# catec/leica_point_cloud_processing

Hardware: AMD Instinct MI355X
Metric: GICP iterations/sec, 5M<->5M scan-vs-CAD (PCL-1.8.1-faithful BFGS GICP) (higher is better)
Workload: dtype f32 transform / f64 accumulate

## Files before the change

### include/mi355x_gicp_debug.h

```cpp
#ifndef MI355X_GICP_DEBUG_H
#define MI355X_GICP_DEBUG_H

#include "mi355x_gicp.h"

#ifdef __cplusplus
extern "C" {
#endif

int mgicp_debug_covariances(mgicp_ctx* ctx, int which, double* out_c6);
int mgicp_debug_source_order(mgicp_ctx* ctx, uint32_t* out, size_t cap);
int mgicp_debug_correspondences(mgicp_ctx* ctx, const float T_cm[16], int* out_tgt, double* out_M6);
int mgicp_debug_correspondences_seeded(mgicp_ctx* ctx, const float T_cm[16], int* out_tgt, double* out_M6);
int mgicp_debug_fdf(mgicp_ctx* ctx, const double x[6], double* f, double g6[6]);
int mgicp_debug_fdf_sums(mgicp_ctx* ctx, const double x[6], double out16[16]);
int mgicp_debug_fdf_sums_run(mgicp_ctx* ctx, const double* xs, int n, double* out16n);
int mgicp_debug_pass_bench(mgicp_ctx* ctx, const double x[6], int npasses, int mode, double* out_ms,
                           double out16[16]);
int mgicp_debug_moments(mgicp_ctx* ctx, const float T_cm[16], double out80[80]);
int mgicp_debug_supers(mgicp_ctx* ctx, int kind, const double* arg, double* out, int cap);
int mgicp_debug_finish_supers(mgicp_ctx* ctx, int nv, const double* rows, long long nsup, long long maxsup,
                              int nranks, double* out);
int mgicp_debug_wave_reduce(mgicp_ctx* ctx, const double* in, int nwaves, double* out_tree, double* out_rs);
int mgicp_debug_trace(mgicp_ctx* ctx, float* out, int max_iters);
#define MGICP_KERNEL_FAMILIES 6
int mgicp_debug_kernel_times(mgicp_ctx* ctx, double out_ms[MGICP_KERNEL_FAMILIES],
                             int out_counts[MGICP_KERNEL_FAMILIES]);
int mgicp_debug_pass_stats(mgicp_ctx* ctx, long long out[9]);
int mgicp_debug_server_time(mgicp_ctx* ctx, double* out_ms, long long* out_passes, long long* out_launches,
                            int reset);
int mgicp_debug_target_cov_slice(mgicp_ctx* ctx, int nranks, int rank, double* out_c6);
int mgicp_debug_vlist_stats(mgicp_ctx* ctx, long long out[8]);
int mgicp_debug_vlist_layout(mgicp_ctx* ctx, double out[24], uint8_t* state, uint32_t* length, uint32_t* offset,
                             size_t cap);
int mgicp_debug_match_stats(mgicp_ctx* ctx, long long out[8]);
int mgicp_set_profiling(mgicp_ctx* ctx, int on);
int mgicp_debug_option(mgicp_ctx* ctx, const char* name, double value);
int mgicp_debug_cache_stats(mgicp_ctx* ctx, long long out[5]);

#ifdef __cplusplus
}
#endif
#endif
// ... 1 lines not shown
```

### leica_point_cloud_processing_amd/_lib.py

```python
from __future__ import annotations

import ctypes
import os
import re

_HERE = os.path.dirname(os.path.abspath(__file__))
LIB_PATH = os.path.join(_HERE, os.environ.get("MGICP_LIB_NAME", "libmgicp.so"))
HEADER_PATH = os.path.join(os.path.dirname(_HERE), "include", "mi355x_gicp.h")
DEBUG_HEADER_PATH = os.path.join(os.path.dirname(_HERE), "include", "mi355x_gicp_debug.h")

MGICP_OK = 0
MGICP_E_INVALID = -1
MGICP_E_TOO_FEW_POINTS = -2
MGICP_E_SOLVER = -3
MGICP_E_NONFINITE = -4
MGICP_E_HIP = -5
MGICP_E_COMM = -6
MGICP_E_NOMEM = -7

MGICP_SOLVER_PCL_BFGS = 0
MGICP_SOLVER_GN = 1
MGICP_KERNEL_FAMILIES = 6


# ... 122 lines not shown
    "mgicp_fpfh_features": (ctypes.c_int, [_P, _P, _SZ, _SZ, _P, _SZ, _P, _SZ, ctypes.c_double, _P, _SZ, _P, _P,
                                            ctypes.POINTER(MgicpFpfhInfo)]),
    "mgicp_match_features": (ctypes.c_int, [_P, _P, _SZ, _SZ, _P, _SZ, _SZ, ctypes.c_double, _P, _P,
                                             ctypes.POINTER(_SZ), ctypes.POINTER(MgicpMatchInfo)]),
    "mgicp_segment_differences": (ctypes.c_int, [_P, _FP, _P, _SZ, _SZ, _P, _SZ, _SZ, ctypes.c_double, _P,
                                                  ctypes.POINTER(_SZ)]),
    "mgicp_voxel_grid": (ctypes.c_int, [_P, _P, _SZ, _SZ, ctypes.c_int, _DP, ctypes.c_int, _P, _SZ,
                                         ctypes.POINTER(_SZ)]),
    "mgicp_euclidean_clusters": (ctypes.c_int, [_P, _P, _SZ, _SZ, ctypes.c_double, _SZ, _SZ, _P, _P, _P,
                                                 ctypes.POINTER(MgicpClusterInfo)]),
    "mgicp_get_unique_id": (ctypes.c_int, [ctypes.c_char_p]),
    "mgicp_comm_init": (ctypes.c_int, [_P, ctypes.c_int, ctypes.c_int, ctypes.c_char_p]),
    "mgicp_comm_attach_shm": (ctypes.c_int, [_P, ctypes.c_char_p, _SZ]),
    "mgicp_comm_attach_xgmi": (ctypes.c_int, [_P, ctypes.c_int]),
    "mgicp_debug_pass_stats": (ctypes.c_int, [_P, ctypes.POINTER(ctypes.c_longlong)]),
    "mgicp_debug_server_time": (ctypes.c_int, [_P, _DP, ctypes.POINTER(ctypes.c_longlong),
                                               ctypes.POINTER(ctypes.c_longlong), ctypes.c_int]),
    "mgicp_debug_target_cov_slice": (ctypes.c_int, [_P, ctypes.c_int, ctypes.c_int, _DP]),
    "mgicp_debug_vlist_stats": (ctypes.c_int, [_P, ctypes.POINTER(ctypes.c_longlong)]),
    "mgicp_debug_match_stats": (ctypes.c_int, [_P, ctypes.POINTER(ctypes.c_longlong)]),
    "mgicp_debug_vlist_layout": (ctypes.c_int, [_P, _DP, _P, _P, _P, _SZ]),
    "mgicp_debug_source_order": (ctypes.c_int, [_P, ctypes.c_void_p, ctypes.c_size_t]),
    "mgicp_debug_covariances": (ctypes.c_int, [_P, ctypes.c_int, _DP]),
    "mgicp_debug_correspondences": (ctypes.c_int, [_P, _FP, _IP, _DP]),
    "mgicp_debug_correspondences_seeded": (ctypes.c_int, [_P, _FP, _IP, _DP]),
    "mgicp_debug_fdf": (ctypes.c_int, [_P, _DP, _DP, _DP]),
    "mgicp_debug_fdf_sums": (ctypes.c_int, [_P, _DP, _DP]),
    "mgicp_debug_fdf_sums_run": (ctypes.c_int, [_P, _DP, ctypes.c_int, _DP]),
    "mgicp_debug_pass_bench": (ctypes.c_int, [_P, _DP, ctypes.c_int, ctypes.c_int, _DP, _DP]),
    "mgicp_debug_moments": (ctypes.c_int, [_P, _FP, _DP]),
# ... 75 lines not shown
```

### leica_point_cloud_processing_amd/csrc/mgicp_ctx.hpp

```cpp
#pragma once
#include <hip/hip_runtime.h>
#include <rccl/rccl.h>

#include <algorithm>
#include <chrono>
#include <cstdio>
#include <cstdlib>
#include <cstring>
#include <memory>
#include <mutex>
#include <string>
#include <vector>

#include "../../include/mi355x_gicp.h"
#include "mgicp_internal.hpp"
#include "pass_memo.hpp"
#include "pcl_bfgs.hpp"
#include "shm_rows.hpp"

using namespace mgicp;

namespace mgicp {

constexpr int kFdfMaxBlocks = 512;
// ... 206 lines not shown
  bool srv_degraded = false;
  unsigned long long srv_next = 0;
  int cus = 0;
  int srv_cus = 0;
  int stall_pass = -1;
  int quit_pass = -1;
  double row_deadline_ms = 500.0;
  double remote_deadline_s = 120.0;
  unsigned long long* h_ptimes = nullptr;
  unsigned long long* d_ptimes = nullptr;
  bool host_rows = true;
  unsigned long long* h_rows = nullptr;
  unsigned long long* d_rows = nullptr;
  size_t rows_cap = 0;
  std::vector<double> row_sums;
  unsigned int pass_idx = 0;
  unsigned long long gather_idx = 0;
  bool have_shm = false;
  shm::Segment shm;
  bool have_xgmi = false;
  DevBuf<unsigned long long> xrows;
  std::vector<void*> xpeer;
  unsigned long long* h_xtot = nullptr;
  unsigned long long* d_xtot = nullptr;
  unsigned int* h_xgen = nullptr;
  unsigned int* d_xgen = nullptr;
  unsigned int xgen = 0;
  unsigned long long xseq = 0;
  hipStream_t xstream = nullptr;
  bool xstream_own = false;
// ... 22 lines not shown
  bool qperm_aux = false;
  DevBuf<uint32_t> aq_keys, aq_keys_sorted, aq_vals;
  DevBuf<unsigned char> aq_scratch;
  DevBuf<unsigned int> aux_cnt;
  DevBuf<uint32_t> knn_fb2;
  bool knn_wave = true;
  bool knn_logged = true;
  DevBuf<uint32_t> knn_fb;
  unsigned int knn_fallbacks = 0;
  DevBuf<float> fpartial;
  unsigned long long match_pairs_per_launch = kMatchPairsPerLaunch;
  long long match_stats[8] = {0, 0, 0, 0, 0, 0, 0, 0};
  bool vlist = true;
  bool fuse_compact = true;
  DevBuf<uint32_t> vl_defer;
  bool vl_stats = false;
  bool vl_valid = false;
  bool vl_alloc = false;
  bool vl_off = false;
  VListView vl{};
  size_t vl_ncells = 0;
  DevBuf<uint32_t> vl_cell, vl_build, vl_bcentre, vl_pend;
  DevBuf<float4> vl_pool;
  DevBuf<unsigned int> vl_ctr;
  uint32_t vl_epoch = 0;
  int vl_groups = 0;
  bool vl_eager = false;
  int vl_cold_groups = 2;
  size_t vl_pool_entries = 0;
  bool tcache_on = false;
// ... 86 lines not shown
  hipEvent_t e = nullptr;
  (void)hipEventCreate(&e);
  return e;
}

struct ProfScope {
  mgicp_ctx* ctx;
  int fam;
  hipEvent_t a = nullptr;
  ProfScope(mgicp_ctx* c, int f) : ctx(c), fam(f) {
    if (ctx->profiling && (fam != kFamFdf || (ctx->prof_tick++ % kProfStride) == 0)) {
      a = ev_get(ctx);
      (void)hipEventRecord(a, ctx->stream);
    }
  }
  ~ProfScope() {
    if (a) {
      hipEvent_t b = ev_get(ctx);
      (void)hipEventRecord(b, ctx->stream);
      ctx->pending.push_back({a, b, fam});
    }
  }
};

Mat4 apply_state(const Vec6& x);
void prof_resolve(mgicp_ctx* ctx);
void cancel_gated(mgicp_ctx* ctx);
void srv_resolve(mgicp_ctx* ctx);
void srv_release(mgicp_ctx* ctx);
int sync(mgicp_ctx* ctx);
int reset_stamps(mgicp_ctx* ctx);
int ensure_host_red(mgicp_ctx* ctx);
CorrSoA corr_soa(mgicp_ctx* ctx);
RowView row_view(const mgicp_ctx* ctx);
int ensure_rows(mgicp_ctx* ctx);
// ... 51 lines not shown
```

### leica_point_cloud_processing_amd/csrc/mgicp_debug.hip

```cpp
#pragma clang fp contract(off)

#include <algorithm>
#include <cstdio>
#include <cstring>
#include <mutex>
#include <string>
#include <vector>

#include "../../include/mi355x_gicp_debug.h"
#include "mgicp_ctx.hpp"

extern "C" {

int mgicp_debug_pass_stats(mgicp_ctx* ctx, long long out[9]) {
  if (!ctx || !out) return MGICP_E_INVALID;
  for (int i = 0; i < kStCount; ++i) out[i] = ctx->st[i];
  return MGICP_OK;
}

int mgicp_debug_server_time(mgicp_ctx* ctx, double* out_ms, long long* out_passes, long long* out_launches,
                            int reset) {
  if (!ctx || !out_ms || !out_passes || !out_launches) return MGICP_E_INVALID;
  *out_ms = ctx->srv_time_ms;
  *out_passes = ctx->srv_time_passes;
  *out_launches = ctx->srv_time_launches;
  if (reset) {
    ctx->srv_time_ms = 0;
    ctx->srv_time_passes = ctx->srv_time_launches = 0;
  }
  return MGICP_OK;
}
// ... 477 lines not shown
    ctx->src_lazy_ready = false;
  } else if (n == "knn_wave") {
    ctx->knn_wave = on;
  } else if (n == "knn_logged") {
    ctx->knn_logged = on;
    ctx->src.have_cov = ctx->tgt.have_cov = false;
    ctx->src_lazy_ready = false;
  } else if (n == "vlist") ctx->vlist = on, ctx->vl_valid = false;
  else if (n == "vlist_cold") ctx->vl_cold_groups = std::max(0, iv), ctx->vl_valid = false;
  else if (n == "vlist_eager") ctx->vl_eager = on, ctx->vl_valid = false;
  else if (n == "vlist_pool") {
    ctx->vl_pool_entries = value >= 1.0 ? static_cast<size_t>(std::min(value, 134217728.0)) : 0;
    ctx->vl_valid = false;
  } else if (n == "vlist_stats") ctx->vl_stats = on;
  else if (n == "fuse_compact") ctx->fuse_compact = on;
  else if (n == "target_cache") ctx->tcache_on = on;
  else if (n == "match_pairs_per_launch")
    ctx->match_pairs_per_launch = value >= 1.0 ? static_cast<unsigned long long>(std::min(value, 9.0e18)) : kMatchPairsPerLaunch;
  else if (n == "bar_cmd") {
    ctx->bar = on;
    if (!on && ctx->bar_cmd) {
      (void)hipFree(ctx->bar_cmd);
      ctx->bar_cmd = nullptr;
    }
    if (on && !ctx->bar_cmd) {
      hipDeviceProp_t prop;
      if (hipGetDeviceProperties(&prop, ctx->device) == hipSuccess && prop.isLargeBar &&
          hipExtMallocWithFlags(reinterpret_cast<void**>(&ctx->bar_cmd), sizeof(PassCmd), hipDeviceMallocFinegrained) ==
              hipSuccess)
        HIPCK(hipMemset(ctx->bar_cmd, 0, sizeof(PassCmd)));
// ... 11 lines not shown
```

### leica_point_cloud_processing_amd/csrc/mgicp_engine.hip

```cpp
#pragma clang fp contract(off)

#include <hip/hip_runtime.h>
#include <rccl/rccl.h>

#include <algorithm>
#include <cmath>
#include <cstdio>
#include <cstdlib>
#include <cstring>
#include <memory>
#include <string>
#include <thread>
#include <vector>

#include "host_upload.hpp"
#include "mgicp_ctx.hpp"
#include "gn_solver.hpp"

using namespace mgicp;

thread_local Graveyard* mgicp::t_new_ctx_grave = nullptr;

namespace {

// ... 95 lines not shown
  }
  ctx->vl.epoch = ctx->vl_epoch;
  ctx->vl.eager = ctx->vl_eager ? 1 : 0;
  ctx->vl.tpts = ctx->tgt.pts.p;
  return MGICP_OK;
}

bool sweep_listed(const mgicp_ctx* ctx) {
  return ctx->vlist && ctx->vl_valid && ctx->vl_alloc && !ctx->vl_off && ctx->vl_groups >= ctx->vl_cold_groups;
}

hipError_t launch_sweep(mgicp_ctx* ctx, const Mat4& T, double thr, bool seeded, const uint32_t* qp,
                        const FusedCompact* fc = nullptr) {
  const size_t p0 = ctx->shard_p0(), p1 = ctx->shard_p1();
  const GridView& g = ctx->tgt.view;
  if (sweep_listed(ctx))
    return launch_vl_sweep(g, ctx->vl, ctx->d_out, p0, p1, T.xf(), thr, seeded ? 1 : 0, ctx->prev_pos.p, ctx->flags.p,
                           ctx->cus, ctx->stream, fc);
  return launch_correspond_wave(g, ctx->d_out, p0, p1, T.xf(), thr, seeded ? 1 : 0, ctx->prev_pos.p, ctx->flags.p, qp,
                                ctx->stream);
}

int report_sweep(mgicp_ctx* ctx) {
  hipStream_t s = ctx->stream;
  if (ctx->vl_stats && sweep_listed(ctx)) {
    unsigned int c3[3];
    HIPCK(hipMemcpyAsync(c3, ctx->vl_ctr.p, 3 * sizeof(unsigned int), hipMemcpyDeviceToHost, s));
    HIPCK(ctx->u64.reserve(64));
    HIPCK(launch_vl_stats(ctx->vl, ctx->vl_ncells, ctx->u64.p, s));
    unsigned long long st[64];
// ... 36 lines not shown
                 ph[14], ph[15], ph[16], ph[17]);
  }
#endif
#if MGICP_CORR_STATS
  {
    unsigned long long st[8];
    HIPCK(hipStreamSynchronize(s));
    HIPCK(corr_stats_take(st));
    std::fprintf(stderr, "[corr-stats] wave scan: queries %llu accepted %llu rejected %llu | per-lane tests/query %.1f "
                 "ranges/query %.1f | lanes left to the per-lane search %llu | union-scan waves %llu of %llu, "
                 "candidates per union wave %.1f\n",
                 st[0], st[1], st[2], st[0] ? double(st[3]) / st[0] : 0.0, st[0] ? double(st[4]) / st[0] : 0.0, st[5],
                 st[7], (st[0] + 63) / 64, st[7] ? double(st[6]) / st[7] : 0.0);
  }
#endif
  return MGICP_OK;
}

struct AlignDrain {
  mgicp_ctx* ctx;
  bool armed = true;
  ~AlignDrain() {
    if (!armed) return;
    const std::string err = ctx->err;
    cancel_gated(ctx);
    (void)hipStreamSynchronize(ctx->stream);
    srv_release(ctx);
    if (!ctx->srv_ev.empty()) srv_resolve(ctx);
    ctx->err = err;
  }
// ... 210 lines not shown
  MGICP_TRACE_AT("corr: lists prepared");
  const bool fused = ctx->fuse_compact && sweep_listed(ctx) && ctx->tgt.have_cov &&
                     !ctx->tgt_cov_pending && !ctx->src_cov_pending &&
                     (ctx->src.have_cov || (ctx->lazy_src_cov && ctx->src_lazy_ready));
  FusedCompact fc{};
  if (fused) {
    HIPCK(ctx->vl_defer.reserve(std::max(chunk_count(ns), 1)));
    fc.cov_s = ctx->src.cov3();
    fc.cov_t = ctx->tgt.cov3();
    fc.R = rot_of(T, G);
    fc.cov_ok = ctx->src.have_cov ? nullptr : ctx->cov_ok.p;
    fc.ccnt = ctx->ccnt.p;
    fc.defer = ctx->vl_defer.p;
    fc.out = corr_soa(ctx);
  }
  {
    ProfScope ps(ctx, kFamCorr);
    HIPCK(launch_sweep(ctx, T, thr, seeded, qp, fused ? &fc : nullptr));
  }
  ctx->seed_valid = true;
  MGICP_TRACE_AT("corr: sweep queued");
  if (int rc = report_sweep(ctx)) return rc;
  {
    int rc = cov_join_all(ctx);
    if (rc) return rc;
    rc = cov_lazy(ctx);
    MGICP_TRACE_AT("corr: lazy covariances queued (sweep drained)");
    if (rc) return rc;
  }
  {
    ProfScope ps(ctx, kFamCompact);
    HIPCK(launch_compact(ctx->d_out, ctx->tgt.view.pts, ctx->src.cov3(), ctx->tgt.cov3(), rot_of(T, G),
                         ctx->prev_pos.p, ctx->flags.p, p0, p1, ctx->ccnt.p, corr_soa(ctx), s,
                         fused ? ctx->vl_defer.p : nullptr, fused ? ctx->vl_ctr.p + 3 : nullptr, ctx->cus));
  }
  ctx->have_corr = true;
  return MGICP_OK;
// ... 188 lines not shown
  ctx->tickets.release();
  ctx->tickets_n = 0;
  ctx->ccnt.release(); ctx->spart.release(); ctx->gath.release(); ctx->msuper.release();
  ctx->prev_pos.release(); ctx->flags.release();
  ctx->vl_cell.release(); ctx->vl_pool.release(); ctx->vl_ctr.release();
  ctx->vl_build.release(); ctx->vl_bcentre.release(); ctx->vl_pend.release(); ctx->vl_defer.release();
  ctx->cov_ok.release(); ctx->cov_need.release();
  ctx->aux_cnt.release(); ctx->knn_fb2.release();
  ctx->tpart.release();
  ctx->tpart_n = 0;
  ctx->corr_f.release(); ctx->corr_d.release();
  ctx->xyz_dev.release();
  if (ctx->mail) (void)hipFree(ctx->mail);
  if (ctx->h_red) (void)hipHostFree(ctx->h_red);
  if (ctx->h_cmd) (void)hipHostFree(ctx->h_cmd);
  if (ctx->h_gtrace) (void)hipHostFree(ctx->h_gtrace);
  if (ctx->h_ptimes) (void)hipHostFree(ctx->h_ptimes);
  if (ctx->h_rows) (void)hipHostFree(ctx->h_rows);
  xgmi_detach(ctx);
  if (ctx->xstream && ctx->xstream_own) (void)hipStreamDestroy(ctx->xstream);
  if (ctx->h_xtot) (void)hipHostFree(ctx->h_xtot);
  if (ctx->have_shm) {
    (void)hipHostUnregister(ctx->shm.base);
    shm::detach(ctx->shm);
    ctx->have_shm = false;
  }
  if (ctx->bar_cmd) (void)hipFree(ctx->bar_cmd);
  if (ctx->h_small) (void)hipHostFree(ctx->h_small);
  prof_resolve(ctx);
  srv_resolve(ctx);
// ... 135 lines not shown
```

### leica_point_cloud_processing_amd/csrc/mgicp_internal.hpp

```cpp
#pragma once
#include <hip/hip_runtime.h>
#include <cstddef>
#include <cstdint>

namespace mgicp {

struct GridView {
  float ox, oy, oz;
  float h, inv_h;
  float slop;
  int nx, ny, nz;
  const uint32_t* cell_start;
  const float4* pts;
  const uint8_t* empty_dist;
  const uint32_t* seed;
  const float4* pairs;
};

#ifndef MGICP_EMPTY_CAP
#define MGICP_EMPTY_CAP 15
#endif
constexpr int kEmptyCap = MGICP_EMPTY_CAP;

struct Cov3 {
// ... 91 lines not shown
  uint32_t* pend;
  uint32_t epoch;
  int eager;
};
struct FusedCompact {
  Cov3 cov_s, cov_t;
  Rot33d R;
  const uint8_t* cov_ok;
  uint32_t* ccnt;
  uint32_t* defer;
  CorrSoA out;
};
hipError_t launch_vl_sweep(const GridView& tgt, const VListView& vl, const float4* src, size_t p0, size_t p1,
                           Xf34 T, double thr, int seeded, uint32_t* nn_pos, uint32_t* flags, int cus,
                           hipStream_t s, const FusedCompact* fc = nullptr);
hipError_t launch_cov_need(const uint32_t* flags, uint8_t* cov_ok, size_t p0, size_t n, uint32_t* list,
                           unsigned int* count, hipStream_t s);
hipError_t launch_vl_stats(const VListView& vl, size_t ncells, unsigned long long* out , hipStream_t s);
size_t     pair_count(size_t n);
hipError_t launch_pairs(const float4* pts, size_t n, float4* out, hipStream_t s);
hipError_t launch_morton_keys(const float4* pts, size_t p0, size_t n, const float lo[3], float inv,
                              uint32_t* keys, uint32_t* vals, hipStream_t s);
hipError_t launch_compact(const float4* src, const float4* tpts, const Cov3& cov_s,
                          const Cov3& cov_t, Rot33d R, const uint32_t* nn_pos,
                          const uint32_t* flags, size_t p0, size_t p1, uint32_t* ccnt, CorrSoA out, hipStream_t s,
                          const uint32_t* defer = nullptr, const unsigned int* defer_count = nullptr, int cus = 0);
hipError_t launch_fdf_soa(const CorrSoA& c, const uint32_t* ccnt, size_t ns, Xf34 A,
                          double* partial, double* spart, int nb, unsigned int* tickets, double* out, int reverse,
                          unsigned long long* done_flag, unsigned long long seq, hipStream_t s,
                          unsigned long long* host_rows = nullptr, unsigned int rstamp = 0);
// ... 122 lines not shown
```

### leica_point_cloud_processing_amd/csrc/mgicp_kernels.hip

```cpp
#pragma clang fp contract(off)

#define MGICP_NN_UNROLL 4
#define MGICP_CORR_WAVES 8
#define MGICP_COV_WAVES 1
#ifndef MGICP_KNN_DIV
#define MGICP_KNN_DIV 0
#endif
#ifndef MGICP_CORR_STATS
#define MGICP_CORR_STATS 0
#endif
#define MGICP_SRV_STAGGER 2
#ifndef MGICP_VL_DIAG
#define MGICP_VL_DIAG 0
#endif
#ifndef MGICP_CORR_PHASES
#define MGICP_CORR_PHASES 0
#endif
constexpr int kRegListBatch = 8;

#include "mgicp_internal.hpp"

#include <hipcub/hipcub.hpp>

#include <algorithm>
// ... 1504 lines not shown
      o.sx[i] = s.x; o.sy[i] = s.y; o.sz[i] = s.z;
      o.qx[i] = w.x; o.qy[i] = w.y; o.qz[i] = w.z;
    }
  }
  if (deferred) {
    if (threadIdx.x == 0) defer[atomicAdd(&v.ctr[3], 1u)] = blockIdx.x;
    return;
  }
  if (threadIdx.x == 0) ccnt[blockIdx.x] = run;
  const uint32_t pad = ((run + 3u) & ~3u) - run;
  if (threadIdx.x < pad) {
    const size_t i = k0 + run + threadIdx.x;
    o.sx[i] = 0.f; o.sy[i] = 0.f; o.sz[i] = 0.f; o.qx[i] = 0.f; o.qy[i] = 0.f; o.qz[i] = 0.f;
    o.m00[i] = 0.0; o.m01[i] = 0.0; o.m02[i] = 0.0; o.m11[i] = 0.0; o.m12[i] = 0.0; o.m22[i] = 0.0;
  }
}

__global__ __launch_bounds__(256) void vl_centre_kernel(GridView tg, VListView v, double thr_c) {
  const unsigned int n = min(v.ctr[1], v.build_cap);
  for (unsigned int i = blockIdx.x * blockDim.x + threadIdx.x; i < n; i += gridDim.x * blockDim.x) {
    uint32_t ix, iy, iz;
    vl_cell_xyz(v, v.build[i], ix, iy, iz);
    const float cx = v.ox + (static_cast<float>(ix) + 0.5f) * v.c;
    const float cy = v.oy + (static_cast<float>(iy) + 0.5f) * v.c;
    const float cz = v.oz + (static_cast<float>(iz) + 0.5f) * v.c;
    NnVisitor vis;
    vis.init(cx, cy, cz, thr_c);
    seed_query(tg, 0, 0xffffffffu, cx, cy, cz, vis);
    if (vis.best != ~0ull) box_search(tg, cx, cy, cz, vis);
    else ring_search(tg, cx, cy, cz, vis);
// ... 2436 lines not shown
    case 25: return knn_cov_k<25>(g, eps, p0, p1, cov, perm, k, fb, fb_count, s, ring_cap, ok, chain, wave_handoff);
    case 30: return knn_cov_k<30>(g, eps, p0, p1, cov, perm, k, fb, fb_count, s, ring_cap, ok, chain, wave_handoff);
    default: break;
  }
  if (k < 1 || k > kMaxK) return hipErrorInvalidValue;
  if (k <= 8) return knn_cov_k<8>(g, eps, p0, p1, cov, perm, k, fb, fb_count, s, ring_cap, ok, chain, wave_handoff);
  if (k <= 16) return knn_cov_k<16>(g, eps, p0, p1, cov, perm, k, fb, fb_count, s, ring_cap, ok, chain, wave_handoff);
  if (k <= 24) return knn_cov_k<24>(g, eps, p0, p1, cov, perm, k, fb, fb_count, s, ring_cap, ok, chain, wave_handoff);
  return knn_cov_k<32>(g, eps, p0, p1, cov, perm, k, fb, fb_count, s, ring_cap, ok, chain, wave_handoff);
}


hipError_t launch_vl_sweep(const GridView& tgt, const VListView& vl, const float4* src, size_t p0, size_t p1,
                           Xf34 T, double thr, int seeded, uint32_t* nn_pos, uint32_t* flags, int cus,
                           hipStream_t s, const FusedCompact* fc) {
  if (p1 <= p0) return hipSuccess;
  hipError_t e = hipMemsetAsync(vl.ctr + 1, 0, 4 * sizeof(unsigned int), s);
  if (e != hipSuccess) return e;
  if (fc)
    vl_query_compact_kernel<<<chunk_count(p1 - p0), 256, 0, s>>>(vl, src, p0, p1 - p0, T, thr, nn_pos, flags, fc->cov_s,
                                                                  fc->cov_t, fc->R, fc->cov_ok, fc->ccnt, fc->defer,
                                                                  fc->out);
  else
    vl_query_kernel<<<nblk(p1 - p0), 256, 0, s>>>(vl, src, p0, p1 - p0, T, thr, nn_pos, flags);
  const double hd = std::sqrt(3.0) * (0.5 * static_cast<double>(vl.c) + static_cast<double>(vl.es));
  const double rc = vl.gate * (1.0 + 1e-5) + 1e-9 + hd;
  const unsigned g = static_cast<unsigned>(std::max(cus, 1));
  vl_centre_kernel<<<4 * g, 256, 0, s>>>(tgt, vl, rc * rc * (1.0 + 1e-5));
  vl_build_kernel<<<8 * g, 64 * kVlWavesS, 0, s>>>(tgt, vl);
  vl_build_large_kernel<<<4 * g, 64 * kVlWaves, 0, s>>>(tgt, vl);
  vl_fallback_kernel<<<8 * g, 256, 0, s>>>(tgt, vl, src, p0, T, thr, seeded, nn_pos, flags);
  return hipGetLastError();
}

constexpr int kCovNeedPer = 16;
__global__ __launch_bounds__(256) void cov_need_kernel(const uint32_t* __restrict__ flags, uint8_t* __restrict__ cov_ok,
                                                       size_t p0, size_t n, uint32_t* __restrict__ list,
                                                       unsigned int* __restrict__ count, int rest) {
  __shared__ unsigned int s_w[4];
// ... 700 lines not shown
      reinterpret_cast<const void*>(&knn_cov_kernel<32>),
      reinterpret_cast<const void*>(&knn_cov2_kernel<5>),
      reinterpret_cast<const void*>(&knn_cov2_kernel<10>),
      reinterpret_cast<const void*>(&knn_cov2_kernel<15>),
      reinterpret_cast<const void*>(&knn_cov2_kernel<20>),
      reinterpret_cast<const void*>(&knn_cov2_kernel<25>),
      reinterpret_cast<const void*>(&knn_cov2_kernel<30>),
      reinterpret_cast<const void*>(&knn_cov2_kernel<8>),
      reinterpret_cast<const void*>(&knn_cov2_kernel<16>),
      reinterpret_cast<const void*>(&knn_cov2_kernel<24>),
      reinterpret_cast<const void*>(&knn_cov2_kernel<32>),
      reinterpret_cast<const void*>(&morton_key_kernel),
      reinterpret_cast<const void*>(&chunk_compact_kernel),
      reinterpret_cast<const void*>(&chunk_compact_list_kernel),
      reinterpret_cast<const void*>(&vl_query_compact_kernel),
      reinterpret_cast<const void*>(&fdf_soa_kernel),
      reinterpret_cast<const void*>(&fdf_soa_gated_kernel),
      reinterpret_cast<const void*>(&fdf_server_kernel<false, kSrvWaves>),
      reinterpret_cast<const void*>(&fdf_server_kernel<true, kSrvWaves>),
      reinterpret_cast<const void*>(&fitness_kernel),
      reinterpret_cast<const void*>(&resolution_kernel),
      reinterpret_cast<const void*>(&radius_keep_kernel),
      reinterpret_cast<const void*>(&reduce_finish_kernel),
      reinterpret_cast<const void*>(&gn_moments_kernel),
      reinterpret_cast<const void*>(&publish_kernel),
      reinterpret_cast<const void*>(&super_reduce_kernel<kRedVals>),
      reinterpret_cast<const void*>(&super_reduce_kernel<kMomVals>),
      reinterpret_cast<const void*>(&finish_supers_kernel<kRedVals>),
      reinterpret_cast<const void*>(&finish_supers_kernel<kMomVals>),
      reinterpret_cast<const void*>(&finite_flags_kernel),
// ... 62 lines not shown
```

### leica_point_cloud_processing_amd/csrc/mgicp_pass.hip

```cpp
#pragma clang fp contract(off)

#include <hip/hip_runtime.h>
#include <rccl/rccl.h>

#include <algorithm>
#include <atomic>
#include <chrono>
#include <cmath>
#include <cstdio>
#include <cstring>

#include "mgicp_ctx.hpp"

using namespace mgicp;

namespace {

std::atomic<int> g_srv_busy[64];

struct Quat { float w, x, y, z; };
Quat quat_axis(float angle, int axis) {
  const float ha = 0.5f * angle;
  float s, c;
  ::sincosf(ha, &s, &c);
// ... 429 lines not shown
    {
      HIPCK(hipHostMalloc(reinterpret_cast<void**>(&ctx->h_ptimes), 2 * 1024 * sizeof(unsigned long long),
                          hipHostMallocMapped | hipHostMallocCoherent));
      HIPCK(hipHostGetDevicePointer(reinterpret_cast<void**>(&ctx->d_ptimes), ctx->h_ptimes, 0));
      std::memset(ctx->h_ptimes, 0, 2 * 1024 * sizeof(unsigned long long));
    }
    {
      HIPCK(hipHostMalloc(reinterpret_cast<void**>(&ctx->h_gtrace), 4 * 1024 * sizeof(unsigned long long),
                          hipHostMallocMapped | hipHostMallocCoherent));
      HIPCK(hipHostGetDevicePointer(reinterpret_cast<void**>(&ctx->d_gtrace), ctx->h_gtrace, 0));
      std::memset(ctx->h_gtrace, 0, 4 * 1024 * sizeof(unsigned long long));
      ctx->host_gt.assign(2 * 1024, 0.0);
    }
#endif
  }
  if (ctx->h_red) return MGICP_OK;
  HIPCK(hipHostMalloc(reinterpret_cast<void**>(&ctx->h_red), 2 * kRedVals * sizeof(double),
                      hipHostMallocMapped | hipHostMallocCoherent));
  HIPCK(hipHostGetDevicePointer(reinterpret_cast<void**>(&ctx->d_h_red), ctx->h_red, 0));
  std::memset(ctx->h_red, 0, 2 * kRedVals * sizeof(double));
  ctx->h_flag = reinterpret_cast<unsigned long long*>(ctx->h_red + kRedVals);
  ctx->d_flag = reinterpret_cast<unsigned long long*>(ctx->d_h_red + kRedVals);
  return MGICP_OK;
}

RowView mgicp::row_view(const mgicp_ctx* ctx) {
  RowView v;
  if (ctx->have_shm) {
    v.h0 = reinterpret_cast<unsigned long long*>(ctx->shm.rows(0));
    v.d0 = reinterpret_cast<unsigned long long*>(ctx->shm_d + ctx->shm.rows_offset_bytes());
// ... 60 lines not shown
        if (shm::row_complete(reinterpret_cast<const uint64_t*>(row), rstamp)) break;
        char msg[192];
        std::snprintf(msg, sizeof(msg),
                      "objective pass finished without publishing its super rows (row %lld of %lld: stamp %08x "
                      "expected, words 0 / 31 carry %08x / %08x)",
                      r, rv.nloc, rstamp, static_cast<unsigned int>(row[0] >> 32),
                      static_cast<unsigned int>(row[31] >> 32));
        return fail(ctx, MGICP_E_HIP, msg);
      }
      if (!own && el > ctx->remote_deadline_s)
        return fail(ctx, MGICP_E_COMM, "another rank did not publish its super rows (shared row segment)");
    }
    shm::row_decode(reinterpret_cast<const uint64_t*>(row), &ctx->row_sums[static_cast<size_t>(r) * kRedVals]);
    return MGICP_OK;
  };
  for (long long r = rv.first; r < rv.first + rv.nloc; ++r) {
    int rc = wait_row(r, true);
    if (rc) return rc;
  }
  t0 = std::chrono::steady_clock::now();
  for (long long r = 0; r < rv.ntot; ++r) {
    if (r >= rv.first && r < rv.first + rv.nloc) continue;
    int rc = wait_row(r, false);
    if (rc) return rc;
  }
  shm::fixed_total(ctx->row_sums.data(), rv.ntot, kRedVals, out);
  return MGICP_OK;
}

int mgicp::ensure_iter_buffers(mgicp_ctx* ctx) {
  const size_t ns = ctx->shard_p1() - ctx->shard_p0();
  const size_t nch = static_cast<size_t>(chunk_count(ns));
  const size_t msup = static_cast<size_t>(ctx->max_supers());
// ... 147 lines not shown
```

### leica_point_cloud_processing_amd/csrc/shm_rows.hpp

```cpp
#pragma once

#include <fcntl.h>
#include <sys/mman.h>
#include <sys/stat.h>
#include <unistd.h>

#include <atomic>
#include <cerrno>
#include <chrono>
#include <cstdint>
#include <cstring>
#include <string>
#include <thread>

namespace mgicp {
namespace shm {

constexpr uint64_t kMagic = 0x31574f5250434947ull;
constexpr int kMaxRanks = 64;
constexpr size_t kHeader = 4096;
constexpr size_t kFlagLine = 64;
constexpr size_t kRowWords = 32;
constexpr int kGathVals = 80;
constexpr size_t kIpcLine = 128;
// ... 161 lines not shown

inline void fixed_total(const double* rows, long long nsup, int nv, double* out) {
  for (int v = 0; v < nv; ++v) {
    double lanes[64];
    for (int l = 0; l < 64; ++l) {
      double a = 0.0;
      for (long long sg = l; sg < nsup; sg += 64) a += rows[static_cast<size_t>(sg) * nv + v];
      lanes[l] = a;
    }
    for (int off = 32; off > 0; off >>= 1)
      for (int i = 0; i < off; ++i) lanes[i] = lanes[i] + lanes[i + off];
    out[v] = lanes[0];
  }
}

inline bool gather_publish_wait(const Segment& s, uint64_t g, double timeout_s) {
  s.flag(s.rank)->store(g, std::memory_order_release);
  const auto t0 = std::chrono::steady_clock::now();
  for (int r = 0; r < s.nranks; ++r) {
    for (unsigned spins = 0; s.flag(r)->load(std::memory_order_acquire) < g; ++spins) {
      if ((spins & 1023u) == 1023u && elapsed_s(t0) > timeout_s) return false;
    }
  }
  return true;
}

}
}
```

### leica_point_cloud_processing_amd/engine.py

```python
from __future__ import annotations

import atexit
import ctypes

import numpy as np

from . import _lib
from .cloud import PointCloudRGB

DBL_MAX = float(np.finfo(np.float64).max)
_LIVE: set = set()
_SHUTTING_DOWN = [False]


@atexit.register
def _mark_shutdown():
    _SHUTTING_DOWN[0] = True


def _cm(T) -> np.ndarray:
    return np.ascontiguousarray(np.asarray(T, dtype=np.float32).T).reshape(16)


def _from_cm(buf) -> np.ndarray:
# ... 340 lines not shown
                    "comm_attach_shm")

    def attach_xgmi(self, on: bool = True):
        self._check(self._lib.mgicp_comm_attach_xgmi(self._h, int(bool(on))), "mgicp_comm_attach_xgmi")

    def detach_shm(self):
        self._check(self._lib.mgicp_comm_attach_shm(self._h, None, 0), "comm_attach_shm(detach)")

    PASS_STATS = ("server_launches", "server_passes", "launched_passes", "takeovers", "bar_commands",
                  "row_allocs", "transport", "server_denied", "memo_hits")

    def pass_stats(self) -> dict:
        out = (ctypes.c_longlong * len(self.PASS_STATS))()
        self._check(self._lib.mgicp_debug_pass_stats(self._h, out), "pass_stats")
        return {k: int(out[i]) for i, k in enumerate(self.PASS_STATS)}

    def server_time(self, reset: bool = False) -> dict:
        ms = ctypes.c_double()
        passes = ctypes.c_longlong()
        launches = ctypes.c_longlong()
        self._check(self._lib.mgicp_debug_server_time(self._h, ctypes.byref(ms), ctypes.byref(passes),
                                                      ctypes.byref(launches), int(reset)), "server_time")
        p = int(passes.value)
        return {"ms": ms.value, "passes": p, "launches": int(launches.value),
                "ms_per_pass": ms.value / p if p else None}

    def debug_target_cov_slice(self, nranks: int, rank: int, n_target: int) -> np.ndarray:
        out = np.zeros((max(1, -(-n_target // nranks)), 6), np.float64)
        cnt = self._check(self._lib.mgicp_debug_target_cov_slice(self._h, int(nranks), int(rank), _dp(out)),
                          "debug_target_cov_slice")
# ... 153 lines not shown
```

Before: 482.5.

## Skip follow-up sweep and covariance join when listed queries resolve all points

```diff
diff --git a/include/mi355x_gicp_debug.h b/include/mi355x_gicp_debug.h
--- a/include/mi355x_gicp_debug.h
+++ b/include/mi355x_gicp_debug.h
@@ -26,6 +26,7 @@
 int mgicp_debug_kernel_times(mgicp_ctx* ctx, double out_ms[MGICP_KERNEL_FAMILIES],
                              int out_counts[MGICP_KERNEL_FAMILIES]);
 int mgicp_debug_pass_stats(mgicp_ctx* ctx, long long out[9]);
+int mgicp_debug_round_stats(mgicp_ctx* ctx, long long out[4]);
 int mgicp_debug_server_time(mgicp_ctx* ctx, double* out_ms, long long* out_passes, long long* out_launches,
                             int reset);
 int mgicp_debug_target_cov_slice(mgicp_ctx* ctx, int nranks, int rank, double* out_c6);
diff --git a/leica_point_cloud_processing_amd/_lib.py b/leica_point_cloud_processing_amd/_lib.py
--- a/leica_point_cloud_processing_amd/_lib.py
+++ b/leica_point_cloud_processing_amd/_lib.py
@@ -160,6 +160,7 @@
     "mgicp_comm_attach_shm": (ctypes.c_int, [_P, ctypes.c_char_p, _SZ]),
     "mgicp_comm_attach_xgmi": (ctypes.c_int, [_P, ctypes.c_int]),
     "mgicp_debug_pass_stats": (ctypes.c_int, [_P, ctypes.POINTER(ctypes.c_longlong)]),
+    "mgicp_debug_round_stats": (ctypes.c_int, [_P, ctypes.POINTER(ctypes.c_longlong)]),
     "mgicp_debug_server_time": (ctypes.c_int, [_P, _DP, ctypes.POINTER(ctypes.c_longlong),
                                                ctypes.POINTER(ctypes.c_longlong), ctypes.c_int]),
     "mgicp_debug_target_cov_slice": (ctypes.c_int, [_P, ctypes.c_int, ctypes.c_int, _DP]),
diff --git a/leica_point_cloud_processing_amd/csrc/mgicp_ctx.hpp b/leica_point_cloud_processing_amd/csrc/mgicp_ctx.hpp
--- a/leica_point_cloud_processing_amd/csrc/mgicp_ctx.hpp
+++ b/leica_point_cloud_processing_amd/csrc/mgicp_ctx.hpp
@@ -244,6 +244,7 @@
   unsigned long long* d_rows = nullptr;
   size_t rows_cap = 0;
   std::vector<double> row_sums;
+  bool rows_running = true;
   unsigned int pass_idx = 0;
   unsigned long long gather_idx = 0;
   bool have_shm = false;
@@ -296,6 +297,12 @@
   bool vlist = true;
   bool fuse_compact = true;
   DevBuf<uint32_t> vl_defer;
+  bool round_fast = true;
+  unsigned long long* h_round = nullptr;
+  unsigned long long* d_round = nullptr;
+  unsigned int round_stamp = 0;
+  const unsigned int* vl_ctr_zero = nullptr;
+  long long round_st[4] = {0, 0, 0, 0};
   bool vl_stats = false;
   bool vl_valid = false;
   bool vl_alloc = false;
@@ -412,11 +419,13 @@
       (void)hipEventRecord(a, ctx->stream);
     }
   }
-  ~ProfScope() {
+  ~ProfScope() { close(); }
+  void close() {
     if (a) {
       hipEvent_t b = ev_get(ctx);
       (void)hipEventRecord(b, ctx->stream);
       ctx->pending.push_back({a, b, fam});
+      a = nullptr;
     }
   }
 };
diff --git a/leica_point_cloud_processing_amd/csrc/mgicp_debug.hip b/leica_point_cloud_processing_amd/csrc/mgicp_debug.hip
--- a/leica_point_cloud_processing_amd/csrc/mgicp_debug.hip
+++ b/leica_point_cloud_processing_amd/csrc/mgicp_debug.hip
@@ -15,6 +15,12 @@
 int mgicp_debug_pass_stats(mgicp_ctx* ctx, long long out[9]) {
   if (!ctx || !out) return MGICP_E_INVALID;
   for (int i = 0; i < kStCount; ++i) out[i] = ctx->st[i];
+  return MGICP_OK;
+}
+
+int mgicp_debug_round_stats(mgicp_ctx* ctx, long long out[4]) {
+  if (!ctx || !out) return MGICP_E_INVALID;
+  for (int i = 0; i < 4; ++i) out[i] = ctx->round_st[i];
   return MGICP_OK;
 }
 
@@ -522,6 +528,8 @@
     ctx->vl_valid = false;
   } else if (n == "vlist_stats") ctx->vl_stats = on;
   else if (n == "fuse_compact") ctx->fuse_compact = on;
+  else if (n == "round_fast") ctx->round_fast = on;
+  else if (n == "rows_running") ctx->rows_running = on;
   else if (n == "target_cache") ctx->tcache_on = on;
   else if (n == "match_pairs_per_launch")
     ctx->match_pairs_per_launch = value >= 1.0 ? static_cast<unsigned long long>(std::min(value, 9.0e18)) : kMatchPairsPerLaunch;
diff --git a/leica_point_cloud_processing_amd/csrc/mgicp_engine.hip b/leica_point_cloud_processing_amd/csrc/mgicp_engine.hip
--- a/leica_point_cloud_processing_amd/csrc/mgicp_engine.hip
+++ b/leica_point_cloud_processing_amd/csrc/mgicp_engine.hip
@@ -133,6 +133,7 @@
                         const FusedCompact* fc = nullptr) {
   const size_t p0 = ctx->shard_p0(), p1 = ctx->shard_p1();
   const GridView& g = ctx->tgt.view;
+  if (sweep_listed(ctx)) ctx->vl_ctr_zero = nullptr;
   if (sweep_listed(ctx))
     return launch_vl_sweep(g, ctx->vl, ctx->d_out, p0, p1, T.xf(), thr, seeded ? 1 : 0, ctx->prev_pos.p, ctx->flags.p,
                            ctx->cus, ctx->stream, fc);
@@ -199,6 +200,26 @@
                  st[7], (st[0] + 63) / 64, st[7] ? double(st[6]) / st[7] : 0.0);
   }
 #endif
+  return MGICP_OK;
+}
+
+int wait_round(mgicp_ctx* ctx, unsigned int stamp, unsigned int c[3]) {
+  auto take = [&]() {
+    for (int i = 0; i < 3; ++i) {
+      const unsigned long long w = __atomic_load_n(ctx->h_round + i, __ATOMIC_ACQUIRE);
+      if (static_cast<unsigned int>(w >> 32) != stamp) return false;
+      c[i] = static_cast<unsigned int>(w);
+    }
+    return true;
+  };
+  const auto t0 = std::chrono::steady_clock::now();
+  for (unsigned spins = 0;; ++spins) {
+    if (take()) return MGICP_OK;
+    if ((spins & 1023u) == 1023u && std::chrono::steady_clock::now() - t0 > std::chrono::milliseconds(500)) break;
+  }
+  int rc = sync(ctx);
+  if (rc) return rc;
+  if (!take()) return fail(ctx, MGICP_E_HIP, "listed sweep finished without publishing its round counters");
   return MGICP_OK;
 }
 
@@ -439,13 +460,38 @@
     fc.defer = ctx->vl_defer.p;
     fc.out = corr_soa(ctx);
   }
+  const bool fast = fused && ctx->round_fast && ctx->h_round && ns > 0;
+  bool clean = false;
+  unsigned int c3[3] = {0, 0, 0};
   {
     ProfScope ps(ctx, kFamCorr);
-    HIPCK(launch_sweep(ctx, T, thr, seeded, qp, fused ? &fc : nullptr));
+    if (fast) {
+      if (++ctx->round_stamp == 0) ctx->round_stamp = 1;
+      const bool zero_ctr = ctx->vl_ctr_zero != ctx->vl_ctr.p;
+      ctx->vl_ctr_zero = nullptr;
+      HIPCK(launch_vl_queries(ctx->vl, ctx->d_out, p0, p1, T.xf(), thr, ctx->prev_pos.p, ctx->flags.p, s, &fc, zero_ctr,
+                              ctx->d_round, ctx->round_stamp));
+      if (int rc = wait_round(ctx, ctx->round_stamp, c3)) return rc;
+      clean = !(c3[0] | c3[1] | c3[2]);
+      if (clean)
+        ctx->vl_ctr_zero = ctx->vl_ctr.p;
+      else
+        HIPCK(launch_vl_follow(ctx->tgt.view, ctx->vl, ctx->d_out, p0, p1, T.xf(), thr, seeded ? 1 : 0, ctx->prev_pos.p,
+                               ctx->flags.p, ctx->cus, s));
+    } else {
+      HIPCK(launch_sweep(ctx, T, thr, seeded, qp, fused ? &fc : nullptr));
+    }
   }
   ctx->seed_valid = true;
   MGICP_TRACE_AT("corr: sweep queued");
   if (int rc = report_sweep(ctx)) return rc;
+  ctx->round_st[clean ? 0 : 1]++;
+  if (c3[2]) ctx->round_st[2]++;
+  if (c3[1]) ctx->round_st[3]++;
+  if (clean) {
+    ctx->have_corr = true;
+    return MGICP_OK;
+  }
   {
     int rc = cov_join_all(ctx);
     if (rc) return rc;
@@ -664,6 +710,7 @@
   if (ctx->mail) (void)hipFree(ctx->mail);
   if (ctx->h_red) (void)hipHostFree(ctx->h_red);
   if (ctx->h_cmd) (void)hipHostFree(ctx->h_cmd);
+  if (ctx->h_round) (void)hipHostFree(ctx->h_round);
   if (ctx->h_gtrace) (void)hipHostFree(ctx->h_gtrace);
   if (ctx->h_ptimes) (void)hipHostFree(ctx->h_ptimes);
   if (ctx->h_rows) (void)hipHostFree(ctx->h_rows);
diff --git a/leica_point_cloud_processing_amd/csrc/mgicp_internal.hpp b/leica_point_cloud_processing_amd/csrc/mgicp_internal.hpp
--- a/leica_point_cloud_processing_amd/csrc/mgicp_internal.hpp
+++ b/leica_point_cloud_processing_amd/csrc/mgicp_internal.hpp
@@ -129,6 +129,12 @@
 hipError_t launch_vl_sweep(const GridView& tgt, const VListView& vl, const float4* src, size_t p0, size_t p1,
                            Xf34 T, double thr, int seeded, uint32_t* nn_pos, uint32_t* flags, int cus,
                            hipStream_t s, const FusedCompact* fc = nullptr);
+hipError_t launch_vl_queries(const VListView& vl, const float4* src, size_t p0, size_t p1, Xf34 T, double thr,
+                             uint32_t* nn_pos, uint32_t* flags, hipStream_t s, const FusedCompact* fc, bool zero_ctr,
+                             unsigned long long* verdict, unsigned int stamp);
+hipError_t launch_vl_follow(const GridView& tgt, const VListView& vl, const float4* src, size_t p0, size_t p1,
+                            Xf34 T, double thr, int seeded, uint32_t* nn_pos, uint32_t* flags, int cus,
+                            hipStream_t s);
 hipError_t launch_cov_need(const uint32_t* flags, uint8_t* cov_ok, size_t p0, size_t n, uint32_t* list,
                            unsigned int* count, hipStream_t s);
 hipError_t launch_vl_stats(const VListView& vl, size_t ncells, unsigned long long* out , hipStream_t s);
diff --git a/leica_point_cloud_processing_amd/csrc/mgicp_kernels.hip b/leica_point_cloud_processing_amd/csrc/mgicp_kernels.hip
--- a/leica_point_cloud_processing_amd/csrc/mgicp_kernels.hip
+++ b/leica_point_cloud_processing_amd/csrc/mgicp_kernels.hip
@@ -1542,6 +1542,14 @@
     o.sx[i] = 0.f; o.sy[i] = 0.f; o.sz[i] = 0.f; o.qx[i] = 0.f; o.qy[i] = 0.f; o.qz[i] = 0.f;
     o.m00[i] = 0.0; o.m01[i] = 0.0; o.m02[i] = 0.0; o.m11[i] = 0.0; o.m12[i] = 0.0; o.m22[i] = 0.0;
   }
+}
+
+__global__ __launch_bounds__(64) void vl_round_publish_kernel(unsigned int* ctr, unsigned long long* host_words,
+                                                              unsigned int stamp) {
+  if (threadIdx.x >= 3) return;
+  const unsigned int c = __hip_atomic_load(ctr + 1 + threadIdx.x, __ATOMIC_RELAXED, __HIP_MEMORY_SCOPE_AGENT);
+  __hip_atomic_store(host_words + threadIdx.x, (static_cast<unsigned long long>(stamp) << 32) | c, __ATOMIC_RELAXED,
+                     __HIP_MEMORY_SCOPE_SYSTEM);
 }
 
 __global__ __launch_bounds__(256) void vl_centre_kernel(GridView tg, VListView v, double thr_c) {
@@ -4008,15 +4016,32 @@
 hipError_t launch_vl_sweep(const GridView& tgt, const VListView& vl, const float4* src, size_t p0, size_t p1,
                            Xf34 T, double thr, int seeded, uint32_t* nn_pos, uint32_t* flags, int cus,
                            hipStream_t s, const FusedCompact* fc) {
+  hipError_t e = launch_vl_queries(vl, src, p0, p1, T, thr, nn_pos, flags, s, fc, true, nullptr, 0);
+  return e != hipSuccess ? e : launch_vl_follow(tgt, vl, src, p0, p1, T, thr, seeded, nn_pos, flags, cus, s);
+}
+
+hipError_t launch_vl_queries(const VListView& vl, const float4* src, size_t p0, size_t p1, Xf34 T, double thr,
+                             uint32_t* nn_pos, uint32_t* flags, hipStream_t s, const FusedCompact* fc, bool zero_ctr,
+                             unsigned long long* verdict, unsigned int stamp) {
   if (p1 <= p0) return hipSuccess;
-  hipError_t e = hipMemsetAsync(vl.ctr + 1, 0, 4 * sizeof(unsigned int), s);
-  if (e != hipSuccess) return e;
+  if (zero_ctr) {
+    hipError_t e = hipMemsetAsync(vl.ctr + 1, 0, 4 * sizeof(unsigned int), s);
+    if (e != hipSuccess) return e;
+  }
   if (fc)
     vl_query_compact_kernel<<<chunk_count(p1 - p0), 256, 0, s>>>(vl, src, p0, p1 - p0, T, thr, nn_pos, flags, fc->cov_s,
                                                                   fc->cov_t, fc->R, fc->cov_ok, fc->ccnt, fc->defer,
                                                                   fc->out);
   else
     vl_query_kernel<<<nblk(p1 - p0), 256, 0, s>>>(vl, src, p0, p1 - p0, T, thr, nn_pos, flags);
+  if (verdict) vl_round_publish_kernel<<<1, 64, 0, s>>>(vl.ctr, verdict, stamp);
+  return hipGetLastError();
+}
+
+hipError_t launch_vl_follow(const GridView& tgt, const VListView& vl, const float4* src, size_t p0, size_t p1,
+                            Xf34 T, double thr, int seeded, uint32_t* nn_pos, uint32_t* flags, int cus,
+                            hipStream_t s) {
+  if (p1 <= p0) return hipSuccess;
   const double hd = std::sqrt(3.0) * (0.5 * static_cast<double>(vl.c) + static_cast<double>(vl.es));
   const double rc = vl.gate * (1.0 + 1e-5) + 1e-9 + hd;
   const unsigned g = static_cast<unsigned>(std::max(cus, 1));
@@ -4747,6 +4772,7 @@
       reinterpret_cast<const void*>(&chunk_compact_kernel),
       reinterpret_cast<const void*>(&chunk_compact_list_kernel),
       reinterpret_cast<const void*>(&vl_query_compact_kernel),
+      reinterpret_cast<const void*>(&vl_round_publish_kernel),
       reinterpret_cast<const void*>(&fdf_soa_kernel),
       reinterpret_cast<const void*>(&fdf_soa_gated_kernel),
       reinterpret_cast<const void*>(&fdf_server_kernel<false, kSrvWaves>),
diff --git a/leica_point_cloud_processing_amd/csrc/mgicp_pass.hip b/leica_point_cloud_processing_amd/csrc/mgicp_pass.hip
--- a/leica_point_cloud_processing_amd/csrc/mgicp_pass.hip
+++ b/leica_point_cloud_processing_amd/csrc/mgicp_pass.hip
@@ -467,6 +467,12 @@
     }
 #endif
   }
+  if (!ctx->h_round) {
+    HIPCK(hipHostMalloc(reinterpret_cast<void**>(&ctx->h_round), 8 * sizeof(unsigned long long),
+                        hipHostMallocMapped | hipHostMallocCoherent));
+    HIPCK(hipHostGetDevicePointer(reinterpret_cast<void**>(&ctx->d_round), ctx->h_round, 0));
+    std::memset(ctx->h_round, 0, 8 * sizeof(unsigned long long));
+  }
   if (ctx->h_red) return MGICP_OK;
   HIPCK(hipHostMalloc(reinterpret_cast<void**>(&ctx->h_red), 2 * kRedVals * sizeof(double),
                       hipHostMallocMapped | hipHostMallocCoherent));
@@ -557,9 +563,18 @@
     shm::row_decode(reinterpret_cast<const uint64_t*>(row), &ctx->row_sums[static_cast<size_t>(r) * kRedVals]);
     return MGICP_OK;
   };
+  static_assert(shm::RunningTotal::kVals == kRedVals, "RunningTotal restates the pass's value count");
+  const bool running = ctx->rows_running && rv.first == 0 && rv.nloc == rv.ntot;
+  shm::RunningTotal rt;
+  if (running) rt.reset();
   for (long long r = rv.first; r < rv.first + rv.nloc; ++r) {
     int rc = wait_row(r, true);
     if (rc) return rc;
+    if (running) rt.add_row(r, &ctx->row_sums[static_cast<size_t>(r) * kRedVals]);
+  }
+  if (running) {
+    rt.finish(out);
+    return MGICP_OK;
   }
   t0 = std::chrono::steady_clock::now();
   for (long long r = 0; r < rv.ntot; ++r) {
diff --git a/leica_point_cloud_processing_amd/csrc/shm_rows.hpp b/leica_point_cloud_processing_amd/csrc/shm_rows.hpp
--- a/leica_point_cloud_processing_amd/csrc/shm_rows.hpp
+++ b/leica_point_cloud_processing_amd/csrc/shm_rows.hpp
@@ -199,6 +199,25 @@
   }
 }
 
+struct RunningTotal {
+  static constexpr int kVals = 16;
+  alignas(64) double lanes[64][kVals];
+  void reset() {
+    for (int l = 0; l < 64; ++l)
+      for (int v = 0; v < kVals; ++v) lanes[l][v] = 0.0;
+  }
+  void add_row(long long r, const double* sums) {
+    double* a = lanes[r & 63];
+    for (int v = 0; v < kVals; ++v) a[v] = a[v] + sums[v];
+  }
+  void finish(double* out) {
+    for (int off = 32; off > 0; off >>= 1)
+      for (int i = 0; i < off; ++i)
+        for (int v = 0; v < kVals; ++v) lanes[i][v] = lanes[i][v] + lanes[i + off][v];
+    for (int v = 0; v < kVals; ++v) out[v] = lanes[0][v];
+  }
+};
+
 inline bool gather_publish_wait(const Segment& s, uint64_t g, double timeout_s) {
   s.flag(s.rank)->store(g, std::memory_order_release);
   const auto t0 = std::chrono::steady_clock::now();
diff --git a/leica_point_cloud_processing_amd/engine.py b/leica_point_cloud_processing_amd/engine.py
--- a/leica_point_cloud_processing_amd/engine.py
+++ b/leica_point_cloud_processing_amd/engine.py
@@ -378,6 +378,13 @@
         out = (ctypes.c_longlong * len(self.PASS_STATS))()
         self._check(self._lib.mgicp_debug_pass_stats(self._h, out), "pass_stats")
         return {k: int(out[i]) for i, k in enumerate(self.PASS_STATS)}
+
+    ROUND_STATS = ("fast", "slow", "deferred", "pending")
+
+    def round_stats(self) -> dict:
+        out = (ctypes.c_longlong * len(self.ROUND_STATS))()
+        self._check(self._lib.mgicp_debug_round_stats(self._h, out), "round_stats")
+        return {k: int(out[i]) for i, k in enumerate(self.ROUND_STATS)}
 
     def server_time(self, reset: bool = False) -> dict:
         ms = ctypes.c_double()
```

New measurement: 504.4, median of 6. 1.05x the previous value.
